# wyhuai/DDNM

Hardware: AMD Instinct MI355X
Metric: restored images/sec @256×256, 100 DDIM steps, 4×SR; 1/2/4/8 GPU (higher is better)
Workload: dtype f32 (3x3 convolutions: fp32 operands carried as hi + lo fp16 halves, three fp16 MFMA products per product, fp32 accumulate -- operand error 2^-22, measured closer to fp64 than the fp32 MFMA kernel; everything else fp32); 1 GPU; celeba_hq.yml SVD sr_bicubic 4x, sigma_y=0, eta=0.85, T_sampling=100, batch_size=8 per GPU (BASELINE configs[1]); global_batch=8, image=3x256x256, parallelism=dp1 (image sharding)

## Files before the change

ddnm_amd/build.py:

```python
import hashlib
import os
import shutil
import subprocess
import sys

HERE = os.path.dirname(os.path.abspath(__file__))
CSRC = os.path.join(HERE, "csrc")
LIB = os.path.join(HERE, "libddnm_hip.so")
STAMP = os.path.join(HERE, ".libddnm_hip.stamp")
OBJ = os.path.join(HERE, "_obj")
SOURCES = ["conv_igemm_f32.hip", "conv_igemm_f16.hip", "conv_s16_persist.hip", "conv_gather_s16.hip", "conv_small_f32.hip", "conv1x1_f16.hip", "conv16.hip", "act16.hip", "attn16.hip", "attn_d512.hip", "attn16_bwd.hip", "gemm_f32.hip", "groupnorm.hip", "misc.hip", "ddnm_step.hip", "fwht.hip", "backward.hip"]
FLAGS = ["--offload-arch=gfx950", "-O3", "-std=c++17", "-fPIC", "-shared", "-Wall", "-Wno-unused-function"]


def _hipcc():
    for c in (os.environ.get("HIPCC"), shutil.which("hipcc"), "/opt/rocm/bin/hipcc"):
        if c and os.path.exists(c):
            return c
    raise RuntimeError("hipcc not found (set HIPCC)")


def _digest():
    h = hashlib.sha256()
    for f in sorted(os.listdir(CSRC)) + ["../../include/ddnm_hip.h"]:
        with open(os.path.join(CSRC, f), "rb") as fh:
            h.update(f.encode() + fh.read())
    h.update(" ".join(FLAGS).encode())
    return h.hexdigest()


LAST_BUILD = {"compiled": False}


def build(force=False, verbose=False):
    dig = _digest()
    LAST_BUILD["compiled"] = False
    if not force and os.path.exists(LIB) and os.path.exists(STAMP) and open(STAMP).read() == dig:
        return LIB
    LAST_BUILD["compiled"] = True
    tmp = LIB + f".tmp{os.getpid()}"
    os.makedirs(OBJ, exist_ok=True)
    hh = hashlib.sha256()
    for f in sorted(os.listdir(CSRC)) + ["../../include/ddnm_hip.h"]:
        if f.endswith(".h"):
            with open(os.path.join(CSRC, f), "rb") as fh:
                hh.update(f.encode() + fh.read())
    hh.update(" ".join(FLAGS).encode())
    cflags = [f for f in FLAGS if f != "-shared"]
    jobs, objs = [], []
    for s in SOURCES:
        h = hashlib.sha256(hh.digest())
        with open(os.path.join(CSRC, s), "rb") as fh:
            h.update(fh.read())
        extra = [f'-DDDNM_BUILD_DIGEST="{dig}"'] if s == "misc.hip" else []
        h.update(" ".join(extra).encode())
        obj = os.path.join(OBJ, f"{s}.{h.hexdigest()[:16]}.o")
        objs.append(obj)
        if force or not os.path.exists(obj):
            jobs.append((s, [_hipcc()] + cflags + extra + ["-c", os.path.join(CSRC, s), "-o", obj + f".tmp{os.getpid()}"], obj))
    if jobs:
        from concurrent.futures import ThreadPoolExecutor

        def run(job):
            s, cmd, obj = job
# ... 34 lines not shown
```

ddnm_amd/csrc/conv_common.h:

```cpp
#pragma once
#include "common.h"

struct ConvArgs {
    ddnm_conv_desc d;
    int Cin, ntaps, Hs, Ws;
    int m_tiles, n_tiles;
    int tiles_x;
    int TW, TW_log2;
    int ksplit;
    float* ws;
};

static inline bool conv_sizes_addressable(const ddnm_conv_desc* d) {
    const int64_t lim = (int64_t)1 << 31;
    const int64_t out_el = (int64_t)d->B * d->Ho * d->Wo * d->Cout;
    const int64_t hs = d->ups ? d->Hin / 2 : d->Hin, ws = d->ups ? d->Win / 2 : d->Win;
    const int64_t cmax = d->C0 > d->C1 ? d->C0 : d->C1;
    const int64_t src_b = (int64_t)d->B * hs * ws * cmax * (d->src_f16 ? 2 : 4);
    const int64_t cout_pad = ((int64_t)d->Cout + 127) / 128 * 128;
    const int64_t w_b = cout_pad * d->ksize * d->ksize * ((int64_t)d->C0 + d->C1) * 4;
    const int64_t sk_el = (int64_t)d->B * d->Ho * d->Wo * (d->SC0 > d->SC1 ? d->SC0 : d->SC1);
    return out_el < lim && src_b < lim && w_b < lim && sk_el < lim;
}

bool conv3x3_s16_persist_eligible(const ConvArgs& p);
int conv3x3_s16_persist_launch(const ConvArgs& p, hipStream_t s);

struct TileMap {
    int img, ty0, tx0, th_unused, TW, TW_log2, flat_base, Wo;
    bool two_d;
    __device__ __forceinline__ void pixel(int r, int& oy, int& ox) const {
        if (two_d) {
            oy = ty0 + (r >> TW_log2);
            ox = tx0 + (r & (TW - 1));
        } else {
            const int pix = flat_base + r;
            oy = pix / Wo;
            ox = pix - oy * Wo;
        }
    }
};

template <int BM>
__device__ __forceinline__ TileMap make_tilemap(const ConvArgs& p, int m_tile) {
    TileMap t;
    const int HWo = p.d.Ho * p.d.Wo;
    const int per_img = HWo / BM;
    t.img = m_tile / per_img;
    const int t_in_img = m_tile - t.img * per_img;
    t.TW = p.TW;
    t.TW_log2 = p.TW_log2;
    t.Wo = p.d.Wo;
    t.two_d = p.tiles_x != 0;
    if (t.two_d) {
        const int ty = t_in_img / p.tiles_x, tx = t_in_img - ty * p.tiles_x;
        t.ty0 = ty * (BM >> p.TW_log2);
        t.tx0 = tx << p.TW_log2;
        t.flat_base = 0;
    } else {
        t.ty0 = t.tx0 = 0;
        t.flat_base = t_in_img * BM;
    }
    return t;
}

template <int WM, int WN, int MT, int NT, bool RES_ALL_UPFRONT = false>
__device__ __forceinline__ void conv_epilogue(const ConvArgs& p, const TileMap& tm, int n_tile, int m_tile, int slice,
                                              f32x16 (&acc)[MT][NT], float* lds, const float acc_scale = 1.f) {
    constexpr int BN = WN * NT * 32;
    const ddnm_conv_desc& d = p.d;
    const int lane = threadIdx.x & 63, wave = threadIdx.x >> 6;
    const int wm = wave / WN, wn = wave % WN;
    const int ncol = lane & 31, rsel = 4 * (lane >> 5);
    const bool partial = p.ksplit > 1;
    float* __restrict__ ws = partial ? p.ws + (size_t)slice * d.B * d.Ho * d.Wo * d.Cout : nullptr;
    const float* __restrict__ res = d.res;
    float* __restrict__ out = d.out;
    const bool want_stats = d.stats_out != nullptr && !partial;
    float cs[NT], cq[NT];
// ... 261 lines not shown
```

ddnm_amd/csrc/conv_gather_s16.hip:

```cpp
#include "conv_common.h"

constexpr int GS_KC = 32;
constexpr int GS_LDH = 72;

template <int WM, int WN, int MT, int NT>
__global__ __launch_bounds__(256) void conv_gather_s16_kernel(const ConvArgs p) {
    constexpr int BM = WM * MT * 32, BN = WN * NT * 32;
    constexpr int AR = BM / 32, BR = BN / 32;
    constexpr int NWB = 3;
    constexpr int WTILE = BN * 128;
    __shared__ __attribute__((aligned(1024))) char lds_all[NWB * WTILE + BM * GS_LDH * 2];
    char* const Bs = lds_all;
    _Float16* const As = reinterpret_cast<_Float16*>(lds_all + NWB * WTILE);

    const ddnm_conv_desc& d = p.d;
    const int tid = threadIdx.x, lane = tid & 63, wave = tid >> 6;
    const int wm = wave / WN, wn = wave % WN;
    const int tile_id = xcd_swizzle(blockIdx.x, gridDim.x);
    const int n_tile = tile_id % p.n_tiles, m_tile = tile_id / p.n_tiles;
    const int slice = blockIdx.y;
    const TileMap tm = make_tilemap<BM>(p, m_tile);
    const int img = tm.img;
    float ascale, inv_ascale;
    s16_operand_scale(d.gn_scale == nullptr ? d.amax_in : nullptr, img, false, ascale, inv_ascale);
// ... 134 lines not shown
            step(it + 1, a_st1, gsc1, gsh1, a_valid1);
        }
        if (it < it_end) step(it, a_st0, gsc0, gsh0, a_valid0);
        asm volatile("s_waitcnt vmcnt(0)" ::: "memory");
    }
    __syncthreads();
    conv_epilogue<WM, WN, MT, NT>(p, tm, n_tile, m_tile, slice, acc, reinterpret_cast<float*>(As), d.acc_scale * inv_ascale);
}

struct PlanGS {
    int tile;
    int BM, BN, ksplit;
};

static bool plan_gs(const ddnm_conv_desc* d, PlanGS* pl) {
    const int HWo = d->Ho * d->Wo;
    const int Cin = d->C0 + d->C1;
    if ((d->ksize != 1 && d->ksize != 3) || (d->stride != 1 && d->stride != 2)) return false;
    if (d->C0 <= 0 || d->C0 % GS_KC || d->C1 % GS_KC || d->out_nchw || d->src_f16 || d->skip0) return false;
    if (d->Cout % 64 || HWo % 64) return false;
    {
        const int64_t px = (int64_t)d->B * (d->ups ? d->Hin / 2 : d->Hin) * (d->ups ? d->Win / 2 : d->Win);
        const int64_t cmax = d->C0 > d->C1 ? d->C0 : d->C1;
        if (px * cmax * 4 >= (int64_t)1 << 31) return false;
    }
    const int nchunks = Cin / GS_KC;
    int tile = 2;
    if (HWo % 128 == 0 && d->Cout % 128 == 0) {
        const long tiles = (long)d->B * (HWo / 128) * (d->Cout / 128);
        if (tiles * nchunks >= 256) tile = 1;
    }
    pl->tile = tile;
    pl->BM = pl->BN = tile == 1 ? 128 : 64;
    const long tiles = (long)d->B * (HWo / pl->BM) * (d->Cout / pl->BN);
    int ks = 1;
    if (d->Cout % 4 == 0 && tiles < 192) {
        ks = (int)((512 + tiles - 1) / tiles);
        if (ks > nchunks) ks = nchunks;
        if (ks > 16) ks = 16;
        if (ks < 1) ks = 1;
    }
    pl->ksplit = ks;
    return true;
}

extern "C" int ddnm_conv_gather_s16_supported(const ddnm_conv_desc* d) {
    PlanGS pl;
    return d && plan_gs(d, &pl) ? 1 : 0;
}

extern "C" int64_t ddnm_conv_gather_s16_workspace_floats(const ddnm_conv_desc* d) {
    PlanGS pl;
    if (!d || !plan_gs(d, &pl)) return DDNM_E_SHAPE;
    return pl.ksplit > 1 ? (int64_t)pl.ksplit * d->B * d->Ho * d->Wo * d->Cout : 0;
}

extern "C" int ddnm_conv_gather_s16_stats_tiles(const ddnm_conv_desc* d) {
    PlanGS pl;
    if (!d || !plan_gs(d, &pl)) return DDNM_E_SHAPE;
    return pl.ksplit > 1 ? splitk_stats_tiles(d) : d->Ho * d->Wo / pl.BM;
}

extern "C" int ddnm_conv_gather_s16_f32(const ddnm_conv_desc* d, void* stream) {
    if (!d || !d->src0 || !d->weight || !d->out) return DDNM_E_BADARG;
    if (d->B <= 0 || d->Cout <= 0 || d->Ho <= 0 || d->Wo <= 0) return DDNM_E_BADARG;
    if (!conv_sizes_addressable(d)) return DDNM_E_SHAPE;
    if (d->C1 > 0 && !d->src1) return DDNM_E_BADARG;
    if (d->gn_scale && !d->gn_shift) return DDNM_E_BADARG;
    if (!(d->acc_scale > 0.f)) return DDNM_E_BADARG;
    if (!d->gn_scale && !d->amax_in) return DDNM_E_BADARG;
    if (d->ups && ((d->Hin | d->Win) & 1)) return DDNM_E_SHAPE;
    if (d->res_ups && ((d->Ho | d->Wo) & 1)) return DDNM_E_SHAPE;
    PlanGS pl;
    if (!plan_gs(d, &pl)) return DDNM_E_SHAPE;
    if (pl.ksplit > 1) {
        const int64_t need = (int64_t)pl.ksplit * d->B * d->Ho * d->Wo * d->Cout;
        if (!d->workspace || d->workspace_floats < need) {
            if (d->stats_out) return DDNM_E_BADARG;
            pl.ksplit = 1;
        }
    }
    ConvArgs p;
    p.d = *d;
    p.Cin = d->C0 + d->C1;
    p.ntaps = d->ksize * d->ksize;
    p.Hs = d->ups ? d->Hin / 2 : d->Hin;
    p.Ws = d->ups ? d->Win / 2 : d->Win;
    p.m_tiles = d->B * (d->Ho * d->Wo / pl.BM);
    p.n_tiles = d->Cout / pl.BN;
    p.TW = 32;
    p.TW_log2 = 5;
    p.tiles_x = 0;
    p.ksplit = pl.ksplit;
    p.ws = d->workspace;
    const dim3 grid(p.m_tiles * p.n_tiles, pl.ksplit);
    hipStream_t s = (hipStream_t)stream;
    if (pl.tile == 1) { DDNM_LAUNCH((conv_gather_s16_kernel<2, 2, 2, 2>), grid, dim3(256), 0, s, p); }
    else { DDNM_LAUNCH((conv_gather_s16_kernel<2, 2, 1, 1>), grid, dim3(256), 0, s, p); }
    if (pl.ksplit > 1) return launch_splitk_reduce(p, s);
    return 0;
}
```

ddnm_amd/csrc/conv_s16_persist.hip:

```cpp
#include <type_traits>

#include "conv_common.h"

typedef unsigned u32x4 __attribute__((ext_vector_type(4)));

namespace {
constexpr int P_WM = 4, P_WN = 2, P_MT = 2, P_NT = 2;
constexpr int P_NTHREADS = 512, P_BN = 128;
constexpr int P_LDH = 72, P_KCH = 32;
constexpr int P_MAXH = 340, P_HWD = 34;
constexpr int P_HCOLS = 8, P_HRPP = P_NTHREADS / P_HCOLS, P_HR = (P_MAXH + P_HRPP - 1) / P_HRPP, P_HSPLIT = (P_HR + 1) / 2;
constexpr int P_BR = P_BN / (P_NTHREADS / 8);
constexpr int P_NWB = 3, P_WTILE = P_BN * 128;
constexpr int P_HBYTES = 2 * P_MAXH * P_LDH * 2;
constexpr int P_NOUT = P_MT * P_NT * 16;
enum { K_MID = 0, K_LAST = 1, K_FIRST = 2 };

constexpr int p_spread(int tap) { return tap == 0 ? 10 : (tap <= 6 ? 9 : 0); }
constexpr int p_first_of(int tap) { return tap == 0 ? 0 : (tap <= 7 ? 10 + 9 * (tap - 1) : P_NOUT); }
static_assert(p_first_of(7) == P_NOUT, "64 values over taps 0..6");
constexpr int p_extra(int kind, int tap, bool has_res, bool ascale) {
    return kind == K_FIRST ? p_spread(tap) + (tap == 0 ? 1 : 0)
                           : (kind == K_LAST ? (tap == 0 ? 4 + (ascale ? 1 : 0) : 0) + (has_res ? p_spread(tap) : 0) : 0);
}
constexpr int p_base(int tap) {
    return (tap == 1 || tap == 2) ? P_BR + P_HSPLIT + 2 : ((tap == 4 || tap == 5) ? P_BR + P_HR - P_HSPLIT : P_BR);
}
constexpr int p_wait(int kind, int tap, bool has_res, bool ascale) {
    return p_base(tap) + (tap >= 1 ? p_extra(kind, tap - 1, has_res, ascale) : 0) + (tap >= 2 ? p_extra(kind, tap - 2, has_res, ascale) : 0);
}
static_assert(p_wait(K_FIRST, 2, true, true) < 64 && p_wait(K_LAST, 2, true, true) < 64, "vmcnt is a 6-bit field");

template <int V>
using ic = std::integral_constant<int, V>;

}

template <bool ASCALE, bool HAS_RES, bool HAS_SKIP = false>
__global__ __launch_bounds__(P_NTHREADS, 1) void conv3x3_s16_persist_kernel(const ConvArgs p, const int total) {
    static_assert(!HAS_SKIP || (ASCALE && !HAS_RES), "a fused shortcut reads a raw operand (bound required) and replaces the residual");
    constexpr int WM = P_WM, WN = P_WN, MT = P_MT, NT = P_NT, BN = P_BN, HR = P_HR, HSPLIT = P_HSPLIT, LDH = P_LDH, KCH = P_KCH;
    constexpr int MAXH = P_MAXH, HWd = P_HWD, NWB = P_NWB, WTILE = P_WTILE, BR = P_BR, NTHREADS = P_NTHREADS;
    __shared__ __attribute__((aligned(1024))) char lds_all[NWB * WTILE + P_HBYTES + WM * BN * 2 * 4];
    char* const Bs = lds_all;
    _Float16* const Hs = reinterpret_cast<_Float16*>(lds_all + NWB * WTILE);
    float* const stat_lds = reinterpret_cast<float*>(lds_all + NWB * WTILE + P_HBYTES);

    const ddnm_conv_desc& d = p.d;
    const int tid = threadIdx.x, lane = tid & 63;
    const int wave = __builtin_amdgcn_readfirstlane(tid >> 6);
    const int wm = wave / WN, wn = wave % WN;
    const int G = gridDim.x;
    const int per_img = (d.Ho * d.Wo) >> 8;
    const int Cout = d.Cout, Wo = d.Wo;

// ... 109 lines not shown
#pragma unroll
    for (int i = 0; i < MT; ++i)
#pragma unroll
        for (int j = 0; j < NT; ++j)
#pragma unroll
            for (int r = 0; r < 16; ++r) acc[i][j][r] = 0.f;
    int a_off[MT];
#pragma unroll
    for (int i = 0; i < MT; ++i) {
        const int m = (wm * MT + i) * 32 + (lane & 31);
        a_off[i] = ((m >> 5) * HWd + (m & 31)) * LDH + (lane >> 5) * 8;
    }
    const int b_frag = ((wn * NT * 32 + (lane & 31)) * 128) + ((((lane >> 5) ^ (((lane & 31) >> 1) & 7))) << 4);
    auto mfma_tap = [&](int tap, int buf, int hbuf) {
        const int ky = tap / 3, kx = tap - 3 * ky;
        const int tap_off = (ky * HWd + kx) * LDH + hbuf * MAXH * LDH;
        const char* bf = Bs + buf * WTILE;
#pragma unroll
        for (int ks = 0; ks < 2; ++ks) {
            half8 ah[MT], al[MT], bh[NT], bl[NT];
#pragma unroll
            for (int i = 0; i < MT; ++i) {
                ah[i] = *reinterpret_cast<const half8*>(Hs + a_off[i] + tap_off + ks * 16);
                al[i] = *reinterpret_cast<const half8*>(Hs + a_off[i] + tap_off + ks * 16 + 32);
            }
#pragma unroll
            for (int j = 0; j < NT; ++j) {
                bh[j] = *reinterpret_cast<const half8*>(bf + ((b_frag ^ (ks << 5)) + j * 32 * 128));
                bl[j] = *reinterpret_cast<const half8*>(bf + ((b_frag ^ ((ks + 2) << 5)) + j * 32 * 128));
            }
#pragma unroll
            for (int i = 0; i < MT; ++i)
#pragma unroll
                for (int j = 0; j < NT; ++j) acc[i][j] = __builtin_amdgcn_mfma_f32_32x32x16_f16(al[i], bh[j], acc[i][j], 0, 0, 0);
#pragma unroll
            for (int i = 0; i < MT; ++i)
#pragma unroll
                for (int j = 0; j < NT; ++j) acc[i][j] = __builtin_amdgcn_mfma_f32_32x32x16_f16(ah[i], bl[j], acc[i][j], 0, 0, 0);
#pragma unroll
            for (int i = 0; i < MT; ++i)
#pragma unroll
                for (int j = 0; j < NT; ++j) acc[i][j] = __builtin_amdgcn_mfma_f32_32x32x16_f16(ah[i], bh[j], acc[i][j], 0, 0, 0);
        }
    };

    const int ncol = lane & 31, rsel = 4 * (lane >> 5);
    const unsigned out_bytes = (unsigned)d.B * d.Ho * Wo * Cout * 4u;
    const __amdgpu_buffer_rsrc_t r_out = __builtin_amdgcn_make_buffer_rsrc(reinterpret_cast<void*>(d.out), 0, out_bytes, 0x00020000);
    const __amdgpu_buffer_rsrc_t r_res = __builtin_amdgcn_make_buffer_rsrc(
        const_cast<void*>(reinterpret_cast<const void*>(d.res)), 0, d.res ? out_bytes : 0u, 0x00020000);
    const __amdgpu_buffer_rsrc_t r_bias = __builtin_amdgcn_make_buffer_rsrc(
        const_cast<void*>(reinterpret_cast<const void*>(d.bias)), 0, d.bias ? (unsigned)Cout * 4u : 0u, 0x00020000);
    const __amdgpu_buffer_rsrc_t r_badd = __builtin_amdgcn_make_buffer_rsrc(
        const_cast<void*>(reinterpret_cast<const void*>(d.badd)), 0, d.badd ? (unsigned)d.B * d.badd_stride * 4u : 0u, 0x00020000);
    const __amdgpu_buffer_rsrc_t r_stats = __builtin_amdgcn_make_buffer_rsrc(
        reinterpret_cast<void*>(d.stats_out), 0, d.stats_out ? (unsigned)p.m_tiles * Cout * 8u : 0u, 0x00020000);
    const unsigned o_lane = (unsigned)(((wm * MT * Wo + rsel) * Cout + wn * NT * 32 + ncol) * 4);
    auto o_soff = [&](unsigned base, int k) {
        const int i = k >> 5, j = (k >> 4) & 1, r = k & 15;
        return base + (unsigned)(((i * Wo + (r & 3) + 8 * (r >> 2)) * Cout + j * 32) * 4);
    };
    auto tile_base = [&]() { return (unsigned)((((t_img * d.Ho + t_ty0) * Wo + t_tx0) * Cout + t_ntile * BN) * 4); };
    const unsigned c_lane = (unsigned)((wn * NT * 32 + ncol) * 4);
    const unsigned st_lane = tid < 2 * BN ? (unsigned)(tid * 4) : HOOB;

    float outv[P_NOUT];
    float addv[NT][2];
#pragma unroll
    for (int k = 0; k < P_NOUT; ++k) outv[k] = 0.f;
#pragma unroll
    for (int j = 0; j < NT; ++j) addv[j][0] = addv[j][1] = 0.f;
    unsigned pend_base = 0, pend_stats = 0;
    unsigned cur_base = 0, cur_stats = 0;
    float epi_cur = d.acc_scale;

    auto finalize = [&]() {
        float cs[NT], cq[NT];
#pragma unroll
        for (int j = 0; j < NT; ++j) {
            cs[j] = cq[j] = 0.f;
            const float add = addv[j][0];
#pragma unroll
            for (int i = 0; i < MT; ++i)
#pragma unroll
                for (int r = 0; r < 16; ++r) {
                    const int k = (i * NT + j) * 16 + r;
                    const float v = acc[i][j][r] * epi_cur + add + (HAS_RES ? outv[k] : 0.f);
                    outv[k] = v;
                    cs[j] += v;
                    cq[j] = __builtin_fmaf(v, v, cq[j]);
                    acc[i][j][r] = 0.f;
                }
            cs[j] += __shfl_xor(cs[j], 32);
            cq[j] += __shfl_xor(cq[j], 32);
        }
        if (lane < 32) {
#pragma unroll
            for (int j = 0; j < NT; ++j) {
                const int c = (wn * NT + j) * 32 + lane;
                stat_lds[(wm * BN + c) * 2 + 0] = cs[j];
                stat_lds[(wm * BN + c) * 2 + 1] = cq[j];
            }
        }
        pend_base = cur_base;
        pend_stats = cur_stats;
    };
    auto store_stats = [&]() {
// ... 160 lines not shown
    bool pending = false;
    for (;;) {
        int c0 = 0;
        if (pending) {
            run_chunk(ic<K_FIRST>{}, 0);
            c0 = 1;
        }
        for (int chunk = c0; chunk < nchunks - 1; ++chunk) run_chunk(ic<K_MID>{}, chunk);
        const int vn = v + G;
        have_next = vn < total;
        const int c_img = t_img, c_ntile = t_ntile;
        const float ascale_cur = ascale_stage;
        const int c_ty0 = t_ty0, c_tx0 = t_tx0;
        if (have_next) {
            tile_of(vn);
            set_hoff();
            gn_img = t_img;
            next_wsoff = (unsigned)t_ntile * BN * w_rowlen;
            next_base = tile_base();
            next_stats = (unsigned)((t_mtile * Cout + t_ntile * BN) * 8);
            n_img_next = t_img;
        }
        {
            const int n_img = t_img, n_ntile = t_ntile;
            t_img = c_img;
            t_ntile = c_ntile;
            run_chunk(ic<K_LAST>{}, nchunks - 1);
            t_img = n_img;
            t_ntile = n_ntile;
        }
        if constexpr (HAS_SKIP) skip_phase(hb ^ 1, ascale_cur, c_img, c_ty0, c_tx0, c_ntile);
        finalize();
        if (!have_next) break;
        v = vn;
        cur_base = next_base;
        cur_stats = next_stats;
        epi_cur = epi_next;
        pending = true;
    }
    __syncthreads();
    store_stats();
#pragma unroll
    for (int k = 0; k < P_NOUT; ++k) __builtin_amdgcn_raw_buffer_store_b32(__float_as_uint(outv[k]), r_out, o_lane, o_soff(pend_base, k), 0);
}

bool conv3x3_s16_persist_eligible(const ConvArgs& p) {
    const ddnm_conv_desc& d = p.d;
    const long tiles = (long)p.m_tiles * p.n_tiles;
    if (d.skip0 && (!d.amax_in || d.res)) return false;
    return p.ksplit == 1 && tiles >= 512 && p.TW == 32 && !d.res_ups && !d.out_nchw && p.Cin / P_KCH >= 2 &&
           (int64_t)d.B * d.Ho * d.Wo * d.Cout * 4 < ((int64_t)1 << 31) && (int64_t)p.m_tiles * d.Cout * 8 < ((int64_t)1 << 31);
}

int conv3x3_s16_persist_launch(const ConvArgs& p, hipStream_t s) {
    int dev = 0, cus = 0;
    if (hipGetDevice(&dev) != hipSuccess || hipDeviceGetAttribute(&cus, hipDeviceAttributeMultiprocessorCount, dev) != hipSuccess || cus <= 0)
        cus = 256;
    const int total = p.m_tiles * p.n_tiles;
    cus -= cus % 8;
    const dim3 grid(total < cus ? total : cus);
    const bool asc = p.d.amax_in != nullptr, res = p.d.res != nullptr;
    if (p.d.skip0) { DDNM_LAUNCH((conv3x3_s16_persist_kernel<true, false, true>), grid, dim3(P_NTHREADS), 0, s, p, total); }
    else if (asc && res) { DDNM_LAUNCH((conv3x3_s16_persist_kernel<true, true>), grid, dim3(P_NTHREADS), 0, s, p, total); }
    else if (asc) { DDNM_LAUNCH((conv3x3_s16_persist_kernel<true, false>), grid, dim3(P_NTHREADS), 0, s, p, total); }
    else if (res) { DDNM_LAUNCH((conv3x3_s16_persist_kernel<false, true>), grid, dim3(P_NTHREADS), 0, s, p, total); }
    else { DDNM_LAUNCH((conv3x3_s16_persist_kernel<false, false>), grid, dim3(P_NTHREADS), 0, s, p, total); }
    return 0;
}
```

ddnm_amd/ops.py:

```python
import ctypes

import numpy as np
import torch

from . import _lib
from ._lib import Conv16Desc, ConvDesc, GemmDesc, StepScalars, check


def _p(t):
    return None if t is None else t.data_ptr()


def _stream():
    return torch.cuda.current_stream().cuda_stream


def _f32c(t, name):
    if t.dtype != torch.float32 or not t.is_contiguous() or not t.is_cuda:
        raise ValueError(f"{name}: expected a contiguous float32 device tensor, got {t.dtype} "
                         f"contiguous={t.is_contiguous()} device={t.device}")
    return t


class KernelTimer:
# ... 15 lines not shown

_timer = None


def set_kernel_timer(t):
    global _timer
    _timer = t


def _launch(fn, d, label, record):
    if _timer is None:
        check(fn(ctypes.byref(d), _stream()), label)
        return
    variant, flops, shape = record()
    e0, e1 = torch.cuda.Event(enable_timing=True), torch.cuda.Event(enable_timing=True)
    e0.record()
    check(fn(ctypes.byref(d), _stream()), label)
    e1.record()
    _timer.records.append((variant, flops, e0, e1))
    _timer.shapes.append(shape)


def max_launch_batch(per_image_bytes, margin=2):
    return max(1, (1 << 31) // int(per_image_bytes) // margin)


CONV_COUT_ALIGN = 128


_conv_ws = {}


def _conv_workspace(device, floats):
    key = (device, _stream())
    ws = _conv_ws.get(key)
    if ws is None or ws.numel() < floats:
        ws = torch.empty(int(floats), dtype=torch.float32, device=device)
        _conv_ws[key] = ws
    return ws


def pack_conv_weight(w, cin_pad=None):
    cout, cin, kh, kw = w.shape
    cin_pad = cin if cin_pad is None else cin_pad
    cout_pad = (cout + CONV_COUT_ALIGN - 1) // CONV_COUT_ALIGN * CONV_COUT_ALIGN
    out = torch.zeros(cout_pad, kh * kw, cin_pad, dtype=torch.float32, device=w.device)
    out[:cout, :, :cin] = w.float().permute(0, 2, 3, 1).reshape(cout, kh * kw, cin)
    return out.contiguous()


import os as _os
_NO_FUSED_GN = False
FORCE_ONE_TILE = False


class Act:
    __slots__ = ("t", "stats", "tiles", "gn")

    def __init__(self, t, stats=None, tiles=0, gn=None):
        self.t, self.stats, self.tiles = t, stats, tiles
        self.gn = gn


def tensor_of(x):
    return x.t if isinstance(x, Act) else x


def _shape_desc(B, H, W, cin, cout, ksize=3, stride=1):
    d = ConvDesc()
    d.B, d.Hin, d.Win, d.C0, d.C1, d.Cout = B, H, W, cin, 0, cout
    d.ksize, d.stride, d.pad, d.Ho, d.Wo = ksize, stride, (ksize // 2 if stride == 1 else 0), H // stride, W // stride
    return d


def conv_fuses_skip(B, H, W, cin, cout):
    return _lib.lib().ddnm_conv2d_f32_fuses_skip(ctypes.byref(_shape_desc(B, H, W, cin, cout))) == 1


def pack_skip_weight(w, f16=False):
    p = pack_conv_weight(w).reshape(-1, w.shape[1]).contiguous()
    return p.to(torch.float16) if f16 else p


def pack_conv_weight_f16(w, cin_pad=None):
    return pack_conv_weight(w, cin_pad=cin_pad).to(torch.float16).contiguous()


def s16_weight_scale(*ws):
    import math
    m = max(float(w.abs().max()) for w in ws)
    if not (m > 0.0) or not math.isfinite(m):
        return 1.0
    return 2.0 ** (13 - math.floor(math.log2(m)))


def pack_conv_weight_s16(w, scale):
    p = pack_conv_weight(w) * float(scale)
    cp, taps, cin = p.shape
    if cin % 32:
        raise ValueError("split packing needs Cin % 32 == 0")
    hi = p.to(torch.float16)
    lo = (p - hi.float()).to(torch.float16)
    hi, lo = hi.view(cp, taps, cin // 32, 1, 32), lo.view(cp, taps, cin // 32, 1, 32)
    return torch.cat([hi, lo], 3).contiguous()


# ... 12 lines not shown


def _s16_act_scale():
    global _S16_ACT_SCALE
    if _S16_ACT_SCALE is None:
        _S16_ACT_SCALE = float(_lib.lib().ddnm_conv3x3_s16_act_scale())
    return _S16_ACT_SCALE


def conv_runs_f16(B, H, W, cin, cout, ksize=3):
    L = _lib.lib()
    d = _shape_desc(B, H, W, cin, cout, ksize)
    return (L.ddnm_conv3x3_f16_supported if ksize == 3 else L.ddnm_conv1x1_f16_supported)(ctypes.byref(d)) == 1


_F16_PREPASS_MIN_COUT = 256
_f16_scratch_buf = {}


def _f16_scratch(device, numel, slot=0):
    key = (device, slot, _stream())
    buf = _f16_scratch_buf.get(key)
    if buf is None or buf.numel() < numel:
        buf = torch.empty(numel, dtype=torch.float16, device=device)
        _f16_scratch_buf[key] = buf
    return buf


AMAX_N = 32
_S16_CHECK = False


def amax_bound(a0, a1=None):
    def src(a):
        if a is None:
            return None, 0, 0
        if isinstance(a, Act) and a.stats is not None:
            B = a.t.shape[0]
            return a.stats, a.stats.numel() // B, 1
        t = tensor_of(a)
        return _f32c(t, "amax source"), t.numel() // t.shape[0], 0
    t0 = tensor_of(a0)
    B = t0.shape[0]
    p0, n0, k0 = src(a0)
    p1, n1, k1 = src(a1)
    out = torch.empty(B * AMAX_N, dtype=torch.float32, device=t0.device)
    check(_lib.lib().ddnm_amax_bound_f32(_p(p0), n0, k0, _p(p1), n1, k1, _p(out), B, _stream()), "ddnm_amax_bound_f32")
    return out


def conv2d(src0, weight, cout, ksize, *, src1=None, bias=None, badd=None, badd_stride=0, res=None, res_ups=False,
           gn=None, gn_silu=True, stride=1, pad=None, ups=False, out=None, out_nchw=False, out_hw=None, tile=0,
           emit_stats=False, weight_f16=None, skip=None, skip_weight=None, skip_weight_f16=None, weight_s16=None,
           raw_amax=None, one_tile=False):
    a_src0, a_src1 = src0, src1
    src0, src1, res = tensor_of(src0), tensor_of(src1), tensor_of(res)
    B, Hs, Ws, C0 = src0.shape
    C1 = 0 if src1 is None else src1.shape[3]
    Hin, Win = (2 * Hs, 2 * Ws) if ups else (Hs, Ws)
    if pad is None:
        pad = ksize // 2
    if out_hw is None:
        Ho, Wo = (Hin // stride, Win // stride)
    else:
        Ho, Wo = out_hw
    if out is None:
        shape = (B, cout, Ho, Wo) if out_nchw else (B, Ho, Wo, cout)
        out = torch.empty(shape, dtype=torch.float32, device=src0.device)
    d = ConvDesc()
    d.src0, d.src1, d.weight = _p(_f32c(src0, "src0")), _p(src1), _p(_f32c(weight, "weight"))
    d.bias, d.badd, d.res = _p(bias), _p(badd), _p(res)
    d.gn_scale, d.gn_shift = (None, None) if gn is None else (_p(gn[0]), _p(gn[1]))
    d.out = _p(out)
    d.B, d.Hin, d.Win, d.C0, d.C1, d.Cout = B, Hin, Win, C0, C1, cout
    d.ksize, d.stride, d.pad, d.Ho, d.Wo = ksize, stride, pad, Ho, Wo
    d.ups, d.gn_silu, d.out_nchw = int(ups), int(gn_silu), int(out_nchw)
    d.badd_stride, d.tile, d.res_ups = badd_stride, tile, int(res_ups)
    d.flags = 1 if (one_tile or FORCE_ONE_TILE) else 0
    L = _lib.lib()
    if out_nchw and cout <= 4 and skip is None and weight_f16 is None and L.ddnm_conv3x3_small_cout_f32_supported(ctypes.byref(d)) == 1:
        _launch(L.ddnm_conv3x3_small_cout_f32, d, "ddnm_conv3x3_small_cout_f32",
                lambda: ("conv3x3_small_cout_f32", 2.0 * B * Ho * Wo * cout * 9 * C0,
                         (B, Ho, Wo, C0, cout, 3, 1, 0, 0, gn is not None, False)))
        return Act(out, None, 0) if emit_stats else out
    f16, f16_1x1 = False, False
    if skip is not None:
        s0, s1 = tensor_of(skip[0]), tensor_of(skip[1])
        d.skip0, d.skip1 = _p(s0), _p(s1)
        d.SC0, d.SC1 = s0.shape[3], (0 if s1 is None else s1.shape[3])
    s16 = (weight_s16 is not None and weight_f16 is None and ksize == 3 and stride == 1
           and (skip is None or (weight_s16[2] is not None and gn is not None and d.SC0 % 32 == 0 and d.SC1 % 32 == 0))
           and L.ddnm_conv3x3_s16_supported(ctypes.byref(d)) == 1)
    s16g = (not s16 and weight_s16 is not None and weight_f16 is None and skip is None and not _NO_S16_GATHER
            and L.ddnm_conv_gather_s16_supported(ctypes.byref(d)) == 1)
    if s16 or s16g:
        d.weight = weight_s16[0].data_ptr()
        d.acc_scale = 1.0 / (float(weight_s16[1]) * _s16_act_scale())
        if gn is None or skip is not None:
            if raw_amax is None:
                raw_amax = amax_bound(*skip) if skip is not None else amax_bound(a_src0, a_src1)
            d.amax_in = raw_amax.data_ptr()
    if weight_f16 is not None:
        if ksize == 3:
            f16 = L.ddnm_conv3x3_f16_supported(ctypes.byref(d)) == 1
            if (not f16 and stride == 1 and not ups and skip is None and not out_nchw and not res_ups
                    and Hs * Ws < 256 and (C0 | C1) % 8 == 0):
                d.ksize, d.pad, d.C0, d.C1, d.gn_scale, d.gn_shift = 1, 0, 9 * (C0 + C1), 0, None, None
                if L.ddnm_conv1x1_f16_supported(ctypes.byref(d)) == 1:
                    col = _f16_scratch(src0.device, B * Hs * Ws * 9 * (C0 + C1), slot=1)
                    check(L.ddnm_im2col3x3_f16(_p(src0), _p(src1), None if gn is None else _p(gn[0]),
                                               None if gn is None else _p(gn[1]), col.data_ptr(), B, Hs, Ws, C0, C1,
                                               int(gn_silu), _stream()), "ddnm_im2col3x3_f16")
                    d.src0, d.src1, d.src_f16 = col.data_ptr(), None, 1
                    f16 = f16_1x1 = True
                    gn = None
                else:
                    d.ksize, d.pad, d.C0, d.C1 = 3, pad, C0, C1
                    d.gn_scale, d.gn_shift = (None, None) if gn is None else (_p(gn[0]), _p(gn[1]))
        elif ksize == 1 and skip is None:
            d.gn_scale, d.gn_shift = None, None
            f16 = f16_1x1 = L.ddnm_conv1x1_f16_supported(ctypes.byref(d)) == 1
            if not f16 and gn is not None:
                d.gn_scale, d.gn_shift = _p(gn[0]), _p(gn[1])
    if f16:
        d.weight = weight_f16.data_ptr()
        if gn is not None and (f16_1x1 or cout >= _F16_PREPASS_MIN_COUT):
            h16 = _f16_scratch(src0.device, B * Hs * Ws * (C0 + C1))
            check(L.ddnm_gn_apply_f16(_p(src0), _p(src1), _p(gn[0]), _p(gn[1]), h16.data_ptr(), B, Hs * Ws, C0, C1,
                                      int(gn_silu), _stream()), "ddnm_gn_apply_f16")
            d.src0, d.src1, d.C0, d.C1 = h16.data_ptr(), None, C0 + C1, 0
            d.gn_scale, d.gn_shift, d.src_f16 = None, None, 1
# ... 513 lines not shown
```

include/ddnm_hip.h:

```cpp
#ifndef DDNM_HIP_H
#define DDNM_HIP_H

#include <stdint.h>

#ifdef __cplusplus
extern "C" {
#endif

#define DDNM_E_BADARG (-1)
#define DDNM_E_SHAPE (-2)

int ddnm_version(void);
const char* ddnm_build_digest(void);
int ddnm_sizeof(int which);
const char* ddnm_error_string(int code);

typedef struct ddnm_conv_desc {
    const float* src0;
    const float* src1;
    const float* weight;
    const float* bias;
    const float* badd;
    const float* res;
    const float* gn_scale;
    const float* gn_shift;
    float* out;
    int32_t B, Hin, Win;
    int32_t C0, C1;
    int32_t Cout;
    int32_t ksize;
    int32_t stride;
    int32_t pad;
    int32_t Ho, Wo;
    int32_t ups;
    int32_t gn_silu;
    int32_t out_nchw;
    int32_t badd_stride;
    int32_t tile;
    float* workspace;
    int64_t workspace_floats;
    int32_t res_ups;
    int32_t src_f16;
    float* stats_out;
    const float* skip0;
    const float* skip1;
    const float* skip_weight;
    int32_t SC0, SC1;
    float acc_scale;
    int32_t flags;
    const float* amax_in;
} ddnm_conv_desc;

#define DDNM_CONV_ONE_TILE 1
#define DDNM_AMAX_N 32

int ddnm_conv2d_f32(const ddnm_conv_desc* d, void* stream);
int ddnm_conv2d_f32_tile_n(const ddnm_conv_desc* d);
int64_t ddnm_conv2d_f32_workspace_floats(const ddnm_conv_desc* d);
int ddnm_conv2d_f32_stats_tiles(const ddnm_conv_desc* d);
int ddnm_conv2d_f32_fuses_skip(const ddnm_conv_desc* d);

int ddnm_conv3x3_small_cout_f32(const ddnm_conv_desc* d, void* stream);
int ddnm_conv3x3_small_cout_f32_supported(const ddnm_conv_desc* d);

int ddnm_conv3x3_f16_f32(const ddnm_conv_desc* d, void* stream);
int ddnm_conv3x3_f16_supported(const ddnm_conv_desc* d);
int64_t ddnm_conv3x3_f16_workspace_floats(const ddnm_conv_desc* d);
int ddnm_conv3x3_f16_stats_tiles(const ddnm_conv_desc* d);

int ddnm_conv3x3_s16_f32(const ddnm_conv_desc* d, void* stream);
int ddnm_conv3x3_s16_supported(const ddnm_conv_desc* d);
int ddnm_conv3x3_s16_persistent(const ddnm_conv_desc* d);
int64_t ddnm_conv3x3_s16_workspace_floats(const ddnm_conv_desc* d);
int ddnm_conv3x3_s16_stats_tiles(const ddnm_conv_desc* d);
float ddnm_conv3x3_s16_act_scale(void);

int ddnm_conv_gather_s16_f32(const ddnm_conv_desc* d, void* stream);
int ddnm_conv_gather_s16_supported(const ddnm_conv_desc* d);
int64_t ddnm_conv_gather_s16_workspace_floats(const ddnm_conv_desc* d);
int ddnm_conv_gather_s16_stats_tiles(const ddnm_conv_desc* d);

int ddnm_conv1x1_f16_f32(const ddnm_conv_desc* d, void* stream);
int ddnm_conv1x1_f16_supported(const ddnm_conv_desc* d);
int64_t ddnm_conv1x1_f16_workspace_floats(const ddnm_conv_desc* d);
int ddnm_conv1x1_f16_stats_tiles(const ddnm_conv_desc* d);

typedef struct ddnm_conv16_desc {
    const void* src;
    const void* weight;
    const float* bias;
    const void* res;
    const void* skip0;
    const void* skip1;
    const void* skip_weight;
    void* out;
    float* stats_out;
    float* workspace;
    int64_t workspace_floats;
    int32_t B, H, W;
    int32_t Cin, Cout;
    int32_t ksize;
    int32_t ups, res_ups;
    int32_t SC0, SC1;
    const void* src1;
    const float* gn_scale;
    const float* gn_shift;
// ... 225 lines not shown
```

Measured before the change: 6.093 images/sec.

## Add batch-folded split-K s16 conv kernel for 8x8 bottleneck 3x3 convs

Adds a dedicated kernel for 3x3 convolutions at 8x8 spatial size. It packs two images' full 8x8 outputs into one 128-row M tile, stages the haloed input once in LDS, and keeps all nine tap weight tiles resident, with split-K over channel chunks feeding the existing reduce. The gather path dispatches to it when eligible, replacing poorly filled per-image tiles at the lowest UNet resolution. It also caches the CU count for the persistent kernel to avoid per-launch driver queries, and tightens a buffer-descriptor bound.

After: 6.164 images/sec (median of 6 runs). +1.2%, better.

```diff
diff --git a/ddnm_amd/build.py b/ddnm_amd/build.py
--- a/ddnm_amd/build.py
+++ b/ddnm_amd/build.py
@@ -9,7 +9,7 @@
 LIB = os.path.join(HERE, "libddnm_hip.so")
 STAMP = os.path.join(HERE, ".libddnm_hip.stamp")
 OBJ = os.path.join(HERE, "_obj")
-SOURCES = ["conv_igemm_f32.hip", "conv_igemm_f16.hip", "conv_s16_persist.hip", "conv_gather_s16.hip", "conv_small_f32.hip", "conv1x1_f16.hip", "conv16.hip", "act16.hip", "attn16.hip", "attn_d512.hip", "attn16_bwd.hip", "gemm_f32.hip", "groupnorm.hip", "misc.hip", "ddnm_step.hip", "fwht.hip", "backward.hip"]
+SOURCES = ["conv_igemm_f32.hip", "conv_igemm_f16.hip", "conv_s16_persist.hip", "conv_gather_s16.hip", "conv_fold_s16.hip", "conv_small_f32.hip", "conv1x1_f16.hip", "conv16.hip", "act16.hip", "attn16.hip", "attn_d512.hip", "attn16_bwd.hip", "gemm_f32.hip", "groupnorm.hip", "misc.hip", "ddnm_step.hip", "fwht.hip", "backward.hip"]
 FLAGS = ["--offload-arch=gfx950", "-O3", "-std=c++17", "-fPIC", "-shared", "-Wall", "-Wno-unused-function"]
 
 
diff --git a/ddnm_amd/csrc/conv_common.h b/ddnm_amd/csrc/conv_common.h
--- a/ddnm_amd/csrc/conv_common.h
+++ b/ddnm_amd/csrc/conv_common.h
@@ -25,6 +25,12 @@
 
 bool conv3x3_s16_persist_eligible(const ConvArgs& p);
 int conv3x3_s16_persist_launch(const ConvArgs& p, hipStream_t s);
+
+struct ConvFoldPlan {
+    int bn, m_tiles, n_tiles, ksplit;
+};
+bool conv_fold_s16_plan(const ddnm_conv_desc* d, ConvFoldPlan* pl);
+int conv_fold_s16_launch(const ddnm_conv_desc* d, const ConvFoldPlan& pl, hipStream_t s);
 
 struct TileMap {
     int img, ty0, tx0, th_unused, TW, TW_log2, flat_base, Wo;
diff --git a/ddnm_amd/csrc/conv_fold_s16.hip b/ddnm_amd/csrc/conv_fold_s16.hip
--- /dev/null
+++ b/ddnm_amd/csrc/conv_fold_s16.hip
@@ -0,0 +1,264 @@
+#include "conv_common.h"
+
+constexpr int FD_KCH = 32;
+constexpr int FD_LDH = 72;
+constexpr int FD_IMGS = 2;
+constexpr int FD_E = 8;
+constexpr int FD_HWD = FD_E + 2;
+constexpr int FD_NP = FD_HWD * FD_HWD;
+constexpr int FD_SLOTS = 128;
+constexpr int FD_BM = FD_IMGS * FD_E * FD_E;
+
+template <int NT>
+__global__ __launch_bounds__(512, 1) void conv3x3_fold_s16_kernel(const ConvArgs p) {
+    constexpr int WM = 4, WN = 2, NTHREADS = 512;
+    constexpr int BM = FD_BM, BN = WN * NT * 32;
+    static_assert(BM == WM * 32, "one 32-row MFMA tile per wave row");
+    constexpr int MAXH = FD_IMGS * FD_SLOTS;
+    constexpr int HROWS_PER_PASS = NTHREADS / 8;
+    constexpr int HR = MAXH / HROWS_PER_PASS;
+    constexpr int HPI = HR / FD_IMGS;
+    constexpr int BR = BN / (NTHREADS / 8);
+    static_assert(BR >= 1, "weight tile / thread mapping");
+    constexpr int NWB = 9;
+    constexpr int WTILE = BN * 128;
+    constexpr int HBYTES = 2 * MAXH * FD_LDH * 2;
+    static_assert(NWB * WTILE + HBYTES <= 160 * 1024, "LDS of one CU");
+    __shared__ __attribute__((aligned(1024))) char lds_all[NWB * WTILE + HBYTES];
+    char* const Bs = lds_all;
+    _Float16* const Hs = reinterpret_cast<_Float16*>(lds_all + NWB * WTILE);
+
+    const ddnm_conv_desc& d = p.d;
+    const int tid = threadIdx.x, lane = tid & 63, wave = tid >> 6;
+    const int wm = wave / WN, wn = wave % WN;
+    int m_tile, g;
+    {
+        const int bid = blockIdx.x, G = p.n_tiles * p.ksplit;
+        if ((G & 7) == 0) {
+            const int k = bid >> 3;
+            m_tile = k % p.m_tiles;
+            g = (k / p.m_tiles) * 8 + (bid & 7);
+        } else {
+            m_tile = bid % p.m_tiles;
+            g = bid / p.m_tiles;
+        }
+    }
+    const int n_tile = g % p.n_tiles, slice = g / p.n_tiles;
+    const int img0 = m_tile * FD_IMGS;
+
+    const int hc = tid & 7, prow = tid >> 3;
+    int hoff[HR];
+#pragma unroll
+    for (int i = 0; i < HR; ++i) {
+        const int img = img0 + i / HPI, hp = prow + HROWS_PER_PASS * (i % HPI);
+        const int hy = hp / FD_HWD, hx = hp - hy * FD_HWD;
+        const int iy = hy - 1, ix = hx - 1;
+        const bool ok = hp < FD_NP && img < d.B && (unsigned)iy < (unsigned)FD_E && (unsigned)ix < (unsigned)FD_E;
+        hoff[i] = ok ? (img * FD_E + iy) * FD_E + ix : -1;
+    }
+    const int lrow = lane >> 3, lpiece = lane & 7;
+    const int wswz = (((wave & 1) << 2) | (lrow >> 1));
+    const unsigned w_rowlen = 9u * (unsigned)p.Cin * 4u;
+    const __amdgpu_buffer_rsrc_t r_w = __builtin_amdgcn_make_buffer_rsrc(
+        const_cast<void*>(reinterpret_cast<const void*>(d.weight)), 0, (unsigned)p.n_tiles * BN * w_rowlen, 0x00020000);
+    const unsigned w_voff = (unsigned)(n_tile * BN + wave * 8 + lrow) * w_rowlen + (unsigned)((lpiece ^ wswz) * 16);
+    auto issue_w = [&](int chunk, int tap, int buf) {
+        char* dst = Bs + buf * WTILE + wave * 1024;
+        const unsigned so = ((unsigned)tap * p.Cin + (unsigned)chunk * FD_KCH) * 4u;
+#pragma unroll
+        for (int j = 0; j < BR; ++j)
+            __builtin_amdgcn_raw_ptr_buffer_load_lds(r_w, (__attribute__((address_space(3))) void*)(dst + j * 8 * 1024), 16, w_voff,
+                                                     so + (unsigned)j * 64u * w_rowlen, 0, 0);
+    };
+
+    const int nchunks = p.Cin / FD_KCH;
+    const int c_begin = (int)((long)nchunks * slice / p.ksplit), c_end = (int)((long)nchunks * (slice + 1) / p.ksplit);
+
+    typedef unsigned u32x4 __attribute__((ext_vector_type(4)));
+    constexpr unsigned HOOB = 0x80000000u;
+    const __amdgpu_buffer_rsrc_t r_s0 = __builtin_amdgcn_make_buffer_rsrc(
+        const_cast<void*>(reinterpret_cast<const void*>(d.src0)), 0, (unsigned)d.B * FD_E * FD_E * d.C0 * 4u, 0x00020000);
+    const __amdgpu_buffer_rsrc_t r_s1 = __builtin_amdgcn_make_buffer_rsrc(
+        const_cast<void*>(reinterpret_cast<const void*>(d.C1 > 0 ? d.src1 : d.src0)), 0,
+        (unsigned)d.B * FD_E * FD_E * (d.C1 > 0 ? d.C1 : d.C0) * 4u, 0x00020000);
+    f32x4 h_st[HR], gsc[FD_IMGS], gsh[FD_IMGS];
+    auto prefetch_halo_img = [&](int chunk, int k, bool live = true) {
+        const int cb = chunk * FD_KCH;
+        const bool first = cb < d.C0;
+        const unsigned cs = first ? d.C0 : d.C1, coff = first ? cb : cb - d.C0;
+        const __amdgpu_buffer_rsrc_t r_s = first ? r_s0 : r_s1;
+#pragma unroll
+        for (int i = 0; i < HR; ++i) {
+            if (i / HPI != k) continue;
+            const unsigned vo = (hoff[i] >= 0 && live) ? ((unsigned)hoff[i] * cs + hc * 4) * 4u : HOOB;
+            h_st[i] = __builtin_bit_cast(f32x4, __builtin_amdgcn_raw_buffer_load_b128(r_s, vo, coff * 4u, 0));
+        }
+        const int img = img0 + k < d.B ? img0 + k : d.B - 1;
+        gsc[k] = *reinterpret_cast<const f32x4*>(d.gn_scale + (size_t)img * p.Cin + cb + hc * 4);
+        gsh[k] = *reinterpret_cast<const f32x4*>(d.gn_shift + (size_t)img * p.Cin + cb + hc * 4);
+    };
+    auto stage_halo_img = [&](int hbuf, int k) {
+#pragma unroll
+        for (int i = 0; i < HR; ++i) {
+            if (i / HPI != k) continue;
+            const int hp = prow + HROWS_PER_PASS * (i % HPI);
+            if (hp < FD_NP) {
+                f32x4 v = h_st[i];
+                if (hoff[i] >= 0) v = gn_act(v, gsc[k], gsh[k], d.gn_silu);
+                split_store(&Hs[(hbuf * MAXH + k * FD_SLOTS + hp) * FD_LDH + hc * 4], v);
+            }
+        }
+    };
+
+    f32x16 acc[NT];
+#pragma unroll
+    for (int j = 0; j < NT; ++j)
+#pragma unroll
+        for (int r = 0; r < 16; ++r) acc[j][r] = 0.f;
+
+    int a_off;
+    {
+        const int m = wm * 32 + (lane & 31);
+        const int k = m / (FD_E * FD_E), px = m % (FD_E * FD_E);
+        a_off = (k * FD_SLOTS + (px / FD_E) * FD_HWD + (px % FD_E)) * FD_LDH + (lane >> 5) * 8;
+    }
+    const int b_frag = ((wn * NT * 32 + (lane & 31)) * 128) + ((((lane >> 5) ^ (((lane & 31) >> 1) & 7))) << 4);
+
+    struct Frag {
+        half8 ah[2], al[2], bh[2][NT], bl[2][NT];
+    };
+    auto load_tap = [&](Frag& f, int tap, int hbuf) {
+        const int ky = tap / 3, kx = tap - 3 * ky;
+        const int tap_off = (ky * FD_HWD + kx) * FD_LDH + hbuf * MAXH * FD_LDH;
+        const char* bf = Bs + tap * WTILE;
+#pragma unroll
+        for (int ks = 0; ks < 2; ++ks) {
+            f.ah[ks] = *reinterpret_cast<const half8*>(Hs + a_off + tap_off + ks * 16);
+            f.al[ks] = *reinterpret_cast<const half8*>(Hs + a_off + tap_off + ks * 16 + 32);
+#pragma unroll
+            for (int j = 0; j < NT; ++j) {
+                f.bh[ks][j] = *reinterpret_cast<const half8*>(bf + ((b_frag ^ (ks << 5)) + j * 32 * 128));
+                f.bl[ks][j] = *reinterpret_cast<const half8*>(bf + ((b_frag ^ ((ks + 2) << 5)) + j * 32 * 128));
+            }
+        }
+    };
+    auto mfma_tap = [&](const Frag& f) {
+#pragma unroll
+        for (int ks = 0; ks < 2; ++ks) {
+#pragma unroll
+            for (int j = 0; j < NT; ++j) acc[j] = __builtin_amdgcn_mfma_f32_32x32x16_f16(f.al[ks], f.bh[ks][j], acc[j], 0, 0, 0);
+#pragma unroll
+            for (int j = 0; j < NT; ++j) acc[j] = __builtin_amdgcn_mfma_f32_32x32x16_f16(f.ah[ks], f.bl[ks][j], acc[j], 0, 0, 0);
+#pragma unroll
+            for (int j = 0; j < NT; ++j) acc[j] = __builtin_amdgcn_mfma_f32_32x32x16_f16(f.ah[ks], f.bh[ks][j], acc[j], 0, 0, 0);
+        }
+    };
+
+    if (c_begin < c_end) {
+        prefetch_halo_img(c_begin, 0);
+        prefetch_halo_img(c_begin, 1);
+        const int last_row = (c_end - c_begin) * 3 - 1;
+        auto issue_row = [&](int q, int row) {
+            q = q < last_row ? q : last_row;
+            const int ch = q / 3, ky = q - 3 * ch;
+#pragma unroll
+            for (int kx = 0; kx < 3; ++kx) issue_w(c_begin + ch, 3 * ky + kx, 3 * row + kx);
+        };
+        issue_row(0, 0);
+        issue_row(1, 1);
+        stage_halo_img(0, 0);
+        stage_halo_img(0, 1);
+        int hb = 0, row0 = 0;
+        for (int chunk = c_begin; chunk < c_end; ++chunk, row0 += 3) {
+            const bool more = chunk + 1 < c_end;
+#pragma unroll
+            for (int ky = 0; ky < 3; ++ky) {
+                if (ky == 0) {
+                    asm volatile("s_waitcnt vmcnt(%0) lgkmcnt(0)" ::"n"(3 * BR) : "memory");
+                } else {
+                    asm volatile("s_waitcnt vmcnt(%0) lgkmcnt(0)" ::"n"(3 * BR + FD_IMGS * (HPI + 2)) : "memory");
+                }
+                __builtin_amdgcn_s_barrier();
+                asm volatile("" ::: "memory");
+                issue_row(row0 + ky + 2, (ky + 2) % 3);
+                asm volatile("" ::: "memory");
+                __builtin_amdgcn_sched_barrier(0);
+                const int nchunk = more ? chunk + 1 : chunk;
+                if (ky == 0) {
+                    prefetch_halo_img(nchunk, 0, more);
+                    prefetch_halo_img(nchunk, 1, more);
+                }
+                if (ky == 2 && more) {
+                    stage_halo_img(hb ^ 1, 0);
+                    stage_halo_img(hb ^ 1, 1);
+                }
+                __builtin_amdgcn_sched_barrier(0);
+                Frag f0, f1;
+                load_tap(f0, 3 * ky, hb);
+                load_tap(f1, 3 * ky + 1, hb);
+                __builtin_amdgcn_sched_barrier(0);
+                mfma_tap(f0);
+                __builtin_amdgcn_sched_barrier(0);
+                load_tap(f0, 3 * ky + 2, hb);
+                __builtin_amdgcn_sched_barrier(0);
+                mfma_tap(f1);
+                mfma_tap(f0);
+            }
+            hb ^= 1;
+        }
+        asm volatile("s_waitcnt vmcnt(0)" ::: "memory");
+    }
+    {
+        float* __restrict__ ws = p.ws + (size_t)slice * d.B * (FD_E * FD_E) * d.Cout;
+        const int ncol = lane & 31, rsel = 4 * (lane >> 5);
+#pragma unroll
+        for (int j = 0; j < NT; ++j) {
+            const unsigned n = (unsigned)(n_tile * BN + (wn * NT + j) * 32 + ncol);
+#pragma unroll
+            for (int r = 0; r < 16; ++r) {
+                const int row = wm * 32 + (r & 3) + 8 * (r >> 2) + rsel;
+                const unsigned pix = (unsigned)(m_tile * BM + row);
+                if ((int)(pix / (FD_E * FD_E)) < d.B) ws[pix * (unsigned)d.Cout + n] = acc[j][r] * d.acc_scale;
+            }
+        }
+    }
+
+}
+
+bool conv_fold_s16_plan(const ddnm_conv_desc* d, ConvFoldPlan* pl) {
+    if (d->flags & DDNM_CONV_NO_FOLD) return false;
+    if (d->ksize != 3 || d->stride != 1 || d->pad != 1) return false;
+    if (d->Hin != FD_E || d->Win != FD_E || d->Ho != FD_E || d->Wo != FD_E) return false;
+    if (d->B < 2 || d->ups || d->out_nchw || d->src_f16 || d->skip0 || !d->gn_scale) return false;
+    if (d->C0 <= 0 || d->C0 % FD_KCH || d->C1 % FD_KCH || d->Cout % 128) return false;
+    if (splitk_stats_tiles(d) <= 0) return false;
+    const int nchunks = (d->C0 + d->C1) / FD_KCH;
+    pl->bn = 64;
+    pl->m_tiles = (d->B + FD_IMGS - 1) / FD_IMGS;
+    pl->n_tiles = d->Cout / pl->bn;
+    int ks = 256 / (pl->m_tiles * pl->n_tiles);
+    if (ks > 8) ks = 8;
+    if (ks > nchunks) ks = nchunks;
+    if (ks < 2) return false;
+    pl->ksplit = ks;
+    return true;
+}
+
+int conv_fold_s16_launch(const ddnm_conv_desc* d, const ConvFoldPlan& pl, hipStream_t s) {
+    ConvArgs p;
+    p.d = *d;
+    p.Cin = d->C0 + d->C1;
+    p.ntaps = 9;
+    p.Hs = d->Hin;
+    p.Ws = d->Win;
+    p.m_tiles = pl.m_tiles;
+    p.n_tiles = pl.n_tiles;
+    p.TW = FD_E;
+    p.TW_log2 = 3;
+    p.tiles_x = 1;
+    p.ksplit = pl.ksplit;
+    p.ws = d->workspace;
+    const dim3 grid(pl.m_tiles * pl.n_tiles * pl.ksplit);
+    DDNM_LAUNCH((conv3x3_fold_s16_kernel<1>), grid, dim3(512), 0, s, p);
+    return launch_splitk_reduce(p, s);
+}
diff --git a/ddnm_amd/csrc/conv_gather_s16.hip b/ddnm_amd/csrc/conv_gather_s16.hip
--- a/ddnm_amd/csrc/conv_gather_s16.hip
+++ b/ddnm_amd/csrc/conv_gather_s16.hip
@@ -210,12 +210,16 @@
 extern "C" int64_t ddnm_conv_gather_s16_workspace_floats(const ddnm_conv_desc* d) {
     PlanGS pl;
     if (!d || !plan_gs(d, &pl)) return DDNM_E_SHAPE;
+    ConvFoldPlan fp;
+    if (conv_fold_s16_plan(d, &fp)) return (int64_t)fp.ksplit * d->B * d->Ho * d->Wo * d->Cout;
     return pl.ksplit > 1 ? (int64_t)pl.ksplit * d->B * d->Ho * d->Wo * d->Cout : 0;
 }
 
 extern "C" int ddnm_conv_gather_s16_stats_tiles(const ddnm_conv_desc* d) {
     PlanGS pl;
     if (!d || !plan_gs(d, &pl)) return DDNM_E_SHAPE;
+    ConvFoldPlan fp;
+    if (conv_fold_s16_plan(d, &fp)) return splitk_stats_tiles(d);
     return pl.ksplit > 1 ? splitk_stats_tiles(d) : d->Ho * d->Wo / pl.BM;
 }
 
@@ -231,6 +235,14 @@
     if (d->res_ups && ((d->Ho | d->Wo) & 1)) return DDNM_E_SHAPE;
     PlanGS pl;
     if (!plan_gs(d, &pl)) return DDNM_E_SHAPE;
+    {
+        ConvFoldPlan fp;
+        if (conv_fold_s16_plan(d, &fp)) {
+            const int64_t need = (int64_t)fp.ksplit * d->B * d->Ho * d->Wo * d->Cout;
+            if (!d->workspace || d->workspace_floats < need) return DDNM_E_BADARG;
+            return conv_fold_s16_launch(d, fp, (hipStream_t)stream);
+        }
+    }
     if (pl.ksplit > 1) {
         const int64_t need = (int64_t)pl.ksplit * d->B * d->Ho * d->Wo * d->Cout;
         if (!d->workspace || d->workspace_floats < need) {
diff --git a/ddnm_amd/csrc/conv_s16_persist.hip b/ddnm_amd/csrc/conv_s16_persist.hip
--- a/ddnm_amd/csrc/conv_s16_persist.hip
+++ b/ddnm_amd/csrc/conv_s16_persist.hip
@@ -1,6 +1,7 @@
 #include <type_traits>
 
 #include "conv_common.h"
+#include <atomic>
 
 typedef unsigned u32x4 __attribute__((ext_vector_type(4)));
 
@@ -216,7 +217,7 @@
     const __amdgpu_buffer_rsrc_t r_bias = __builtin_amdgcn_make_buffer_rsrc(
         const_cast<void*>(reinterpret_cast<const void*>(d.bias)), 0, d.bias ? (unsigned)Cout * 4u : 0u, 0x00020000);
     const __amdgpu_buffer_rsrc_t r_badd = __builtin_amdgcn_make_buffer_rsrc(
-        const_cast<void*>(reinterpret_cast<const void*>(d.badd)), 0, d.badd ? (unsigned)d.B * d.badd_stride * 4u : 0u, 0x00020000);
+        const_cast<void*>(reinterpret_cast<const void*>(d.badd)), 0, d.badd ? ((unsigned)(d.B - 1) * d.badd_stride + d.Cout) * 4u : 0u, 0x00020000);
     const __amdgpu_buffer_rsrc_t r_stats = __builtin_amdgcn_make_buffer_rsrc(
         reinterpret_cast<void*>(d.stats_out), 0, d.stats_out ? (unsigned)p.m_tiles * Cout * 8u : 0u, 0x00020000);
     const unsigned o_lane = (unsigned)(((wm * MT * Wo + rsel) * Cout + wn * NT * 32 + ncol) * 4);
@@ -483,10 +484,21 @@
            (int64_t)d.B * d.Ho * d.Wo * d.Cout * 4 < ((int64_t)1 << 31) && (int64_t)p.m_tiles * d.Cout * 8 < ((int64_t)1 << 31);
 }
 
+static int persist_cu_count() {
+    constexpr int MAXDEV = 64;
+    static std::atomic<int> cache[MAXDEV];
+    int dev = 0;
+    if (hipGetDevice(&dev) != hipSuccess || dev < 0 || dev >= MAXDEV) return 256;
+    int cus = cache[dev].load(std::memory_order_relaxed);
+    if (cus == 0) {
+        if (hipDeviceGetAttribute(&cus, hipDeviceAttributeMultiprocessorCount, dev) != hipSuccess || cus <= 0) cus = 256;
+        cache[dev].store(cus, std::memory_order_relaxed);
+    }
+    return cus;
+}
+
 int conv3x3_s16_persist_launch(const ConvArgs& p, hipStream_t s) {
-    int dev = 0, cus = 0;
-    if (hipGetDevice(&dev) != hipSuccess || hipDeviceGetAttribute(&cus, hipDeviceAttributeMultiprocessorCount, dev) != hipSuccess || cus <= 0)
-        cus = 256;
+    int cus = persist_cu_count();
     const int total = p.m_tiles * p.n_tiles;
     cus -= cus % 8;
     const dim3 grid(total < cus ? total : cus);
diff --git a/ddnm_amd/ops.py b/ddnm_amd/ops.py
--- a/ddnm_amd/ops.py
+++ b/ddnm_amd/ops.py
@@ -91,6 +91,7 @@
 import os as _os
 _NO_FUSED_GN = False
 FORCE_ONE_TILE = False
+FORCE_NO_FOLD = False
 
 
 class Act:
@@ -209,7 +210,7 @@
 def conv2d(src0, weight, cout, ksize, *, src1=None, bias=None, badd=None, badd_stride=0, res=None, res_ups=False,
            gn=None, gn_silu=True, stride=1, pad=None, ups=False, out=None, out_nchw=False, out_hw=None, tile=0,
            emit_stats=False, weight_f16=None, skip=None, skip_weight=None, skip_weight_f16=None, weight_s16=None,
-           raw_amax=None, one_tile=False):
+           raw_amax=None, one_tile=False, no_fold=False):
     a_src0, a_src1 = src0, src1
     src0, src1, res = tensor_of(src0), tensor_of(src1), tensor_of(res)
     B, Hs, Ws, C0 = src0.shape
@@ -233,7 +234,7 @@
     d.ksize, d.stride, d.pad, d.Ho, d.Wo = ksize, stride, pad, Ho, Wo
     d.ups, d.gn_silu, d.out_nchw = int(ups), int(gn_silu), int(out_nchw)
     d.badd_stride, d.tile, d.res_ups = badd_stride, tile, int(res_ups)
-    d.flags = 1 if (one_tile or FORCE_ONE_TILE) else 0
+    d.flags = (1 if (one_tile or FORCE_ONE_TILE) else 0) | (2 if (no_fold or FORCE_NO_FOLD) else 0)
     L = _lib.lib()
     if out_nchw and cout <= 4 and skip is None and weight_f16 is None and L.ddnm_conv3x3_small_cout_f32_supported(ctypes.byref(d)) == 1:
         _launch(L.ddnm_conv3x3_small_cout_f32, d, "ddnm_conv3x3_small_cout_f32",
diff --git a/include/ddnm_hip.h b/include/ddnm_hip.h
--- a/include/ddnm_hip.h
+++ b/include/ddnm_hip.h
@@ -52,6 +52,7 @@
 } ddnm_conv_desc;
 
 #define DDNM_CONV_ONE_TILE 1
+#define DDNM_CONV_NO_FOLD 2
 #define DDNM_AMAX_N 32
 
 int ddnm_conv2d_f32(const ddnm_conv_desc* d, void* stream);
```
